# bayesiains/nflows

Hardware: AMD Instinct MI355X
Metric: log_prob samples/sec (dim=64, K=8, 32-layer RQ-NSF) + max |fwd∘inv − x| (higher is better)
Workload: dtype f32 (inputs, outputs, spline arithmetic, accumulation; conditioner GEMMs: every fp32 operand carried as 3 f16 pieces = 33 significand bits, i.e. at the reference's own fp32 operand width, 5 cross products per multiply-add -- 3 on the f16 MFMA, the 2 at the 2^-22 level from the pieces' high bytes on

## Files before the change

nflows_amd/csrc/f16x3_gemm.hpp:

```cpp
#pragma once

#include "bf16x3_gemm.hpp"

namespace nfa {

typedef _Float16 f16x8 __attribute__((ext_vector_type(8)));
typedef int i32x8 __attribute__((ext_vector_type(8)));

namespace k8x {

constexpr int kScaleA = 119, kScaleB = 127;

#ifdef NFA_ABL_NO_MFMA
#define NFA_K8X_F16(a, b, c) (c)
#define NFA_K8X_BF8(a, b, c) (c)
#else
#define NFA_K8X_F16(a, b, c) __builtin_amdgcn_mfma_f32_32x32x16_f16(a, b, c, 0, 0, 0)
#define NFA_K8X_BF8(a, b, c) __builtin_amdgcn_mfma_scale_f32_32x32x64_f8f6f4(a, b, c, 1, 1, 0, kScaleA, 0, kScaleB)
#endif

__device__ __forceinline__ void request_stage(WeightStream& sm) {
    const int dst_slot = sm.slot >= 1 ? sm.slot - 1 : kRing - 1;
    const char* stage = reinterpret_cast<const char*>(sm.w) + (size_t)sm.fetch * (kStageVec4 * 16);
    const __amdgpu_buffer_rsrc_t rsrc =
        __builtin_amdgcn_make_buffer_rsrc(const_cast<char*>(stage), (short)0, kStageVec4 * 16, 0x00020000);
    const int wave = __builtin_amdgcn_readfirstlane(sm.tid >> 6);
    char* slot = reinterpret_cast<char*>(sm.ring) + dst_slot * (kStageVec4 * 16) + wave * (kWave * 16);
    const unsigned lane_off = (unsigned)sm.tid * 16u;
#pragma unroll
    for (int i = 0; i < 3; ++i)
        __builtin_amdgcn_raw_ptr_buffer_load_lds(rsrc, (__attribute__((address_space(3))) void*)(slot + i * kBlock * 16), 16,
                                                 lane_off, i * kBlock * 16, 0, 0);
    sm.fetch = (sm.fetch + 1 == sm.num_stages) ? 0 : sm.fetch + 1;
}

template <int WAVES, int SUB>
__device__ __forceinline__ void request_stage(WeightStream& sm) {
    static_assert(WAVES == 4 || WAVES == 8, "narrow or wide");
    if constexpr (WAVES == 4) {
        request_stage(sm);
    } else if constexpr (SUB == 0) {
        const int dst_half = sm.slot >= 2 ? sm.slot - 2 : sm.slot + 2 * kRing - 2;
        const char* stage = reinterpret_cast<const char*>(sm.w) + (size_t)sm.fetch * (kStageVec4 * 16);
        const __amdgpu_buffer_rsrc_t rsrc =
            __builtin_amdgcn_make_buffer_rsrc(const_cast<char*>(stage), (short)0, 2 * kStageVec4 * 16, 0x00020000);
        const int wave = __builtin_amdgcn_readfirstlane(sm.tid >> 6);
        char* slot = reinterpret_cast<char*>(sm.ring) + dst_half * (kStageVec4 * 16) + wave * (kWave * 16);
        const unsigned lane_off = (unsigned)sm.tid * 16u;
#pragma unroll
        for (int i = 0; i < 3; ++i)
            __builtin_amdgcn_raw_ptr_buffer_load_lds(rsrc, (__attribute__((address_space(3))) void*)(slot + i * WAVES * kWave * 16),
                                                     16, lane_off, i * WAVES * kWave * 16, 0, 0);
        sm.fetch = (sm.fetch + 2 == sm.num_stages) ? 0 : sm.fetch + 2;
    }
}
template <int WAVES, int SUB>
__device__ __forceinline__ void stream_advance(WeightStream& sm) {
    if constexpr (WAVES == 4) {
        stream_advance(sm);
    } else {
        if constexpr (SUB == 1) asm volatile("s_waitcnt vmcnt(3)\n\ts_waitcnt lgkmcnt(0)\n\ts_barrier" ::: "memory");
        sm.slot = (sm.slot + 1 == 2 * kRing) ? 0 : sm.slot + 1;
    }
}

struct Pieces {
    uvec4 h, l, r;
};

#define NFA_K8X_ASM asm volatile

#define NFA_K8X_SPLIT_REST                                                  \
    "v_fma_mixlo_f16 %1, %3, 1.0, 0 op_sel_hi:[0,0,0]\n\t"                  \
    "v_fma_mixhi_f16 %1, %4, 1.0, 0 op_sel_hi:[0,0,0]\n\t"                  \
    "v_fma_mix_f32 %3, %3, 1.0, -%1 op_sel_hi:[0,0,1]\n\t"                  \
    "v_fma_mix_f32 %4, %4, 1.0, -%1 op_sel:[0,0,1] op_sel_hi:[0,0,1]\n\t"   \
    "v_fma_mixlo_f16 %2, %3, %8, 0 op_sel_hi:[0,0,0]\n\t"                   \
    "v_fma_mixhi_f16 %2, %4, %8, 0 op_sel_hi:[0,0,0]"
template <bool RELU = false>
__device__ __forceinline__ void split3_scaled(float v0, float v1, float scale, unsigned& hi, unsigned& lo, unsigned& rr) {
#if defined(NFA_K8X_NO_ASM)
    typedef _Float16 h2 __attribute__((ext_vector_type(2)));
    if (RELU) {
        v0 = __builtin_isnan(v0) ? v0 : (v0 > 0.0f ? v0 : 0.0f);
        v1 = __builtin_isnan(v1) ? v1 : (v1 > 0.0f ? v1 : 0.0f);
    }
    const float x0 = v0 * scale, x1 = v1 * scale;
    const h2 h = {(_Float16)x0, (_Float16)x1};
    const float t0 = x0 - (float)h[0], t1 = x1 - (float)h[1];
    const h2 l = {(_Float16)t0, (_Float16)t1};
    const h2 r = {(_Float16)((t0 - (float)l[0]) * 256.0f), (_Float16)((t1 - (float)l[1]) * 256.0f)};
    hi = __builtin_bit_cast(unsigned, h);
    lo = __builtin_bit_cast(unsigned, l);
    rr = __builtin_bit_cast(unsigned, r);
#else
    unsigned h, l, r;
    float t0, t1;
    if constexpr (RELU)
        NFA_K8X_ASM(
            "v_maximum3_f32 %3, %5, 0, 0\n\t"
            "v_maximum3_f32 %4, %6, 0, 0\n\t"
            "v_fma_mixlo_f16 %0, %3, %7, 0 op_sel_hi:[0,0,0]\n\t"
            "v_fma_mixhi_f16 %0, %4, %7, 0 op_sel_hi:[0,0,0]\n\t"
            "v_fma_mix_f32 %3, %3, %7, -%0 op_sel_hi:[0,0,1]\n\t"
            "v_fma_mix_f32 %4, %4, %7, -%0 op_sel:[0,0,1] op_sel_hi:[0,0,1]\n\t"
            NFA_K8X_SPLIT_REST
            : "=&v"(h), "=&v"(l), "=&v"(r), "=&v"(t0), "=&v"(t1)
            : "v"(v0), "v"(v1), "v"(scale), "s"(256.0f));
    else
        NFA_K8X_ASM(
            "v_fma_mixlo_f16 %0, %5, %7, 0 op_sel_hi:[0,0,0]\n\t"
            "v_fma_mixhi_f16 %0, %6, %7, 0 op_sel_hi:[0,0,0]\n\t"
            "v_fma_mix_f32 %3, %5, %7, -%0 op_sel_hi:[0,0,1]\n\t"
            "v_fma_mix_f32 %4, %6, %7, -%0 op_sel:[0,0,1] op_sel_hi:[0,0,1]\n\t"
            NFA_K8X_SPLIT_REST
            : "=&v"(h), "=&v"(l), "=&v"(r), "=&v"(t0), "=&v"(t1)
            : "v"(v0), "v"(v1), "v"(scale), "s"(256.0f));
    hi = h;
    lo = l;
    rr = r;
#endif
}
#undef NFA_K8X_SPLIT_REST

__device__ __forceinline__ i32x8 bf8_operand(const Pieces& p0, const Pieces& p1) {
    constexpr unsigned kHigh = 0x07050301u;
    i32x8 b;
    b[0] = (int)__builtin_amdgcn_perm(p0.r[1], p0.r[0], kHigh);
    b[1] = (int)__builtin_amdgcn_perm(p0.r[3], p0.r[2], kHigh);
    b[2] = (int)__builtin_amdgcn_perm(p0.h[1], p0.h[0], kHigh);
    b[3] = (int)__builtin_amdgcn_perm(p0.h[3], p0.h[2], kHigh);
    b[4] = (int)__builtin_amdgcn_perm(p1.r[1], p1.r[0], kHigh);
    b[5] = (int)__builtin_amdgcn_perm(p1.r[3], p1.r[2], kHigh);
    b[6] = (int)__builtin_amdgcn_perm(p1.h[1], p1.h[0], kHigh);
    b[7] = (int)__builtin_amdgcn_perm(p1.h[3], p1.h[2], kHigh);
    return b;
}

template <bool RELU, bool WB = true>
__device__ __forceinline__ void tile_to_pieces(const f32x16& a, float scale, Pieces& p0, Pieces& p1) {
    if constexpr (WB) asm volatile("s_nop 7\n\ts_nop 3" : : "v"(a));
#pragma unroll
    for (int q2 = 0; q2 < 8; ++q2) {
        unsigned h, l, r;
        split3_scaled<RELU>(a[q2 * 2], a[q2 * 2 + 1], scale, h, l, r);
        if (q2 < 4) {
            p0.h[q2] = h;
            p0.l[q2] = l;
            p0.r[q2] = r;
        } else {
            p1.h[q2 - 4] = h;
            p1.l[q2 - 4] = l;
            p1.r[q2 - 4] = r;
        }
    }
}

__device__ __forceinline__ i32x8 join_x(vec4f lo, vec4f hi) {
    const uvec4 a = __builtin_bit_cast(uvec4, lo), b = __builtin_bit_cast(uvec4, hi);
    return i32x8{(int)a[0], (int)a[1], (int)a[2], (int)a[3], (int)b[0], (int)b[1], (int)b[2], (int)b[3]};
}

struct Lead {
    vec4f h0, l0, h1, l1;
};
__device__ __forceinline__ Lead read_lead(const vec4f* stage) {
    return Lead{stage[0 * 64], stage[1 * 64], stage[2 * 64], stage[3 * 64]};
}

#define NFA_K8X_FENCE() __builtin_amdgcn_sched_barrier(0)

template <bool LAST, int WAVES = 4, int SUB = 0>
__device__ __forceinline__ void stage_kmajor(f32x16& acc0, f32x16& acc1, const Pieces& b0, const Pieces& b1, const i32x8& bx,
                                             WeightStream& sm, int lane, Lead& lead) {
    request_stage<WAVES, SUB>(sm);
    const vec4f* cur = sm.ring + sm.slot * kStageVec4 + lane;
    const f16x8 bh0 = __builtin_bit_cast(f16x8, b0.h), bl0 = __builtin_bit_cast(f16x8, b0.l);
    const f16x8 bh1 = __builtin_bit_cast(f16x8, b1.h), bl1 = __builtin_bit_cast(f16x8, b1.l);
    const vec4f x0l = cur[4 * 64], x0h = cur[5 * 64];
    const vec4f h0 = cur[6 * 64], l0 = cur[7 * 64], h1 = cur[8 * 64], l1 = cur[9 * 64], x1l = cur[10 * 64], x1h = cur[11 * 64];
    NFA_K8X_FENCE();
    {
        const f16x8 ah0 = __builtin_bit_cast(f16x8, lead.h0), al0 = __builtin_bit_cast(f16x8, lead.l0);
        const f16x8 ah1 = __builtin_bit_cast(f16x8, lead.h1), al1 = __builtin_bit_cast(f16x8, lead.l1);
        acc0 = NFA_K8X_F16(ah0, bl0, acc0);
        acc0 = NFA_K8X_F16(al0, bh0, acc0);
        acc0 = NFA_K8X_F16(ah0, bh0, acc0);
        acc0 = NFA_K8X_F16(ah1, bl1, acc0);
        acc0 = NFA_K8X_F16(al1, bh1, acc0);
        acc0 = NFA_K8X_F16(ah1, bh1, acc0);
        acc0 = NFA_K8X_BF8(join_x(x0l, x0h), bx, acc0);
    }
    const f16x8 ah0 = __builtin_bit_cast(f16x8, h0), al0 = __builtin_bit_cast(f16x8, l0);
    const f16x8 ah1 = __builtin_bit_cast(f16x8, h1), al1 = __builtin_bit_cast(f16x8, l1);
    const i32x8 ax = join_x(x1l, x1h);
    acc1 = NFA_K8X_F16(ah0, bl0, acc1);
    acc1 = NFA_K8X_F16(al0, bh0, acc1);
    acc1 = NFA_K8X_F16(ah0, bh0, acc1);
    NFA_K8X_FENCE();
    stream_advance<WAVES, SUB>(sm);
    if constexpr (!LAST) lead = read_lead(sm.ring + sm.slot * kStageVec4 + lane);
    NFA_K8X_FENCE();
    acc1 = NFA_K8X_F16(ah1, bl1, acc1);
    acc1 = NFA_K8X_F16(al1, bh1, acc1);
    acc1 = NFA_K8X_F16(ah1, bh1, acc1);
    acc1 = NFA_K8X_BF8(ax, bx, acc1);
}

template <int NKS, int WAVES, class PairFn>
__device__ __forceinline__ void gemm_kmajor_pairs(f32x16 (&acc)[4], WeightStream& sm, int lane, PairFn&& pair) {
    static_assert(NKS % 2 == 0, "pairs of k-steps");
    Lead lead = read_lead(sm.ring + sm.slot * kStageVec4 + lane);
#pragma unroll
    for (int pr = 0; pr < NKS / 2; ++pr) {
        Pieces b0, b1;
        pair(pr, b0, b1);
        const i32x8 bx = bf8_operand(b0, b1);
        stage_kmajor<false, WAVES, 0>(acc[0], acc[1], b0, b1, bx, sm, lane, lead);
        if (pr + 1 < NKS / 2) stage_kmajor<false, WAVES, 1>(acc[2], acc[3], b0, b1, bx, sm, lane, lead);
        else stage_kmajor<true, WAVES, 1>(acc[2], acc[3], b0, b1, bx, sm, lane, lead);
    }
}

template <int NKS, int WAVES = 4>
__device__ __forceinline__ void gemm_kmajor(f32x16 (&acc)[4], const Pieces (&p)[8], WeightStream& sm, int lane) {
    gemm_kmajor_pairs<NKS, WAVES>(acc, sm, lane, [&](int pr, Pieces& b0, Pieces& b1) {
        b0 = p[2 * pr];
        b1 = p[2 * pr + 1];
    });
}

template <int WAVES = 4>
__device__ __forceinline__ void gemm_kmajor_relu(f32x16 (&acc)[4], const f32x16 (&src)[4], float scale, WeightStream& sm,
                                                 int lane) {
    gemm_kmajor_pairs<8, WAVES>(acc, sm, lane, [&](int pr, Pieces& b0, Pieces& b1) {
        if (pr == 0) tile_to_pieces<true, true>(src[pr], scale, b0, b1);
        else tile_to_pieces<true, false>(src[pr], scale, b0, b1);
    });
}

}
}
```

nflows_amd/csrc/rqs_fused8.hpp:

```cpp
#pragma once

#include "rqs_math.hpp"

namespace nfa {

template <bool INVERSE, int KT = 8, bool DBG = false>
struct FusedSteps {
    static_assert(KT >= 2 && KT <= 32, "2 .. 32 bins (8 and 10 keep their own maximum / sum chains)");
    static constexpr int kNumSlices = KT + 3;
    static constexpr int kWalkSlices = 3 + (KT - 1);
    static constexpr int kBinSlices = INVERSE ? 9 : 7;
    static constexpr int kFinishSlices = kWalkSlices + 6 + kBinSlices + 1;
    static constexpr int kFirstWalkSlices = 0;
    static constexpr bool kInverse = INVERSE;

    float ew[KT], eh[KT];
    float sd[KT - 1];
    float x;
    float kl2e, kappa, tail_s;
    float m_w, m_h, den_w, den_h, tw_, th_;
    float aw, ah, kw, kh, kwn, khn;
    unsigned long long take;
    float cw0, cw1, ch0, ch1, u0, u1, d0, d1;
    float y, lad;
    int status;
    float t3, t4;
    float in_w, in_h, r_w, r_den, delta, s_, th, t1mt, den, t0, t1, t2, t5;
    int kbin;

    template <int A, int B>
    __device__ __forceinline__ static float half_sum(const float (&e)[KT]) {
        float s0 = e[A], s1 = B - A > 1 ? e[A + 1] : 0.0f;
#pragma unroll
        for (int i = A + 2; i < B; i += 2) {
            s0 += e[i];
            if (i + 1 < B) s1 += e[i + 1];
        }
        return B - A > 1 ? s0 + s1 : s0;
    }
    template <int S>
    __device__ __forceinline__ void numerators(float (&e)[KT], float& den_, float& m, float& t) {
        if constexpr (S == 0) {
            if constexpr (KT == 8 || KT == 10) {
                m = __builtin_fmaxf(__builtin_fmaxf(e[0], e[1]), e[2]);
                m = __builtin_fmaxf(__builtin_fmaxf(m, e[3]), e[4]);
                m = __builtin_fmaxf(__builtin_fmaxf(m, e[5]), e[6]);
                if constexpr (KT == 10) m = __builtin_fmaxf(__builtin_fmaxf(m, e[7]), e[8]);
                m = __builtin_fmaxf(m, e[KT - 1]) * kl2e;
            } else {
                m = e[0];
#pragma unroll
                for (int i = 1; i + 1 < KT; i += 2) m = __builtin_fmaxf(__builtin_fmaxf(m, e[i]), e[i + 1]);
                if constexpr (KT % 2 == 0) m = __builtin_fmaxf(m, e[KT - 1]);
                m *= kl2e;
            }
        } else if constexpr (S < 1 + KT) {
            e[S - 1] = __builtin_amdgcn_exp2f(__builtin_fmaf(e[S - 1], kl2e, -m));
        } else if constexpr (KT == 8 || KT == 10) {
            if constexpr (S == 1 + KT) {
                t = (e[0] + e[1]) + (e[2] + e[3]);
            } else {
                den_ = t + ((e[4] + e[5]) + (e[6] + e[7]));
                if constexpr (KT == 10) den_ += e[8] + e[9];
            }
        } else {
            constexpr int H = KT / 2;
            if constexpr (S == 1 + KT) t = half_sum<0, H>(e);
            else den_ = t + half_sum<H, KT>(e);
        }
    }
    template <int S>
    __device__ __forceinline__ void num_w() { numerators<S>(ew, den_w, m_w, tw_); }
    template <int S>
    __device__ __forceinline__ void num_h() { numerators<S>(eh, den_h, m_h, th_); }

    template <int PART>
    __device__ __forceinline__ void derivative(float u, float& d, const RqsDev& sp) {
        if constexpr (PART == 0) {
            t3 = u * kappa;
            t4 = __builtin_amdgcn_exp2f(-__builtin_fabsf(u * kl2e));
        } else if constexpr (PART == 1) {
            const float u1p = 1.0f + t4;
            const float c = t4 - (u1p - 1.0f);
            const float lg = __builtin_fmaf(__builtin_amdgcn_logf(u1p), 0.693147182464599609375f, sp.min_d);
            t4 = __builtin_fmaf(c, __builtin_amdgcn_rcpf(u1p), lg);
        } else {
            d = __builtin_fmaxf(t3, 0.0f) + t4;
        }
    }

    __device__ __forceinline__ void walk_select(float next_lower, float cand_u0, float cand_u1) {
        unsigned long long next;
        asm("v_cmp_ge_f32 %6, %7, %8\n\t"
            "v_cndmask_b32 %0, %0, %9, %15\n\t"
            "v_cndmask_b32 %1, %1, %10, %15\n\t"
            "v_cndmask_b32 %2, %2, %11, %15\n\t"
            "v_cndmask_b32 %3, %3, %12, %15\n\t"
            "v_cndmask_b32 %4, %4, %13, %15\n\t"
            "v_cndmask_b32 %5, %5, %14, %15"
            : "+v"(cw0), "+v"(cw1), "+v"(ch0), "+v"(ch1), "+v"(u0), "+v"(u1), "=&s"(next)
            : "v"(x), "v"(next_lower), "v"(kw), "v"(kwn), "v"(kh), "v"(khn), "v"(cand_u0), "v"(cand_u1), "s"(take));
        take = next;
    }

    template <int S>
    __device__ __forceinline__ void finish(const RqsDev& sp) {
        constexpr int W = kWalkSlices, D0 = W, BE = D0 + 6, LAST = BE + kBinSlices;
        static_assert(LAST + 1 == kFinishSlices, "slice map");
        const float B = sp.right;
        if constexpr (S == 0) {
            const float r0 = __builtin_amdgcn_rcpf(den_w);
            const float r = __builtin_fmaf(__builtin_fmaf(-den_w, r0, 1.0f), r0, r0);
            aw = r * (sp.span_w * sp.om_w);
        } else if constexpr (S == 1) {
            const float r0 = __builtin_amdgcn_rcpf(den_h);
            const float r = __builtin_fmaf(__builtin_fmaf(-den_h, r0, 1.0f), r0, r0);
            ah = r * (sp.span_w * sp.om_h);
        } else if constexpr (S == 2) {
            const float k1w = -B + __builtin_fmaf(ew[0], aw, sp.span_w * sp.min_w);
            const float k1h = -B + __builtin_fmaf(eh[0], ah, sp.span_w * sp.min_h);
            cw0 = -B;
            ch0 = -B;
            cw1 = k1w;
            ch1 = k1h;
            u0 = tail_s;
            u1 = sd[0];
            kw = k1w;
            kh = k1h;
            kwn = k1w + __builtin_fmaf(ew[1], aw, sp.span_w * sp.min_w);
            khn = k1h + __builtin_fmaf(eh[1], ah, sp.span_w * sp.min_h);
            asm("v_cmp_ge_f32 %0, %1, %2" : "=s"(take) : "v"(x), "v"(INVERSE ? k1h : k1w));
            if constexpr (DBG) kbin = 0;
        } else if constexpr (S < W) {
            constexpr int I = S - 2;
            if constexpr (DBG) kbin = (x >= (INVERSE ? kh : kw)) ? I : kbin;
            float kw2 = B, kh2 = B;
            if constexpr (I + 1 < KT - 1) {
                kw2 = kwn + __builtin_fmaf(ew[I + 1], aw, sp.span_w * sp.min_w);
                kh2 = khn + __builtin_fmaf(eh[I + 1], ah, sp.span_w * sp.min_h);
            }
            walk_select(INVERSE ? khn : kwn, sd[I - 1], I < KT - 1 ? sd[I < KT - 1 ? I : 0] : tail_s);
            kw = kwn;
            kh = khn;
            kwn = kw2;
            khn = kh2;
        } else if constexpr (S < D0 + 3) {
            derivative<S - D0>(u0, d0, sp);
        } else if constexpr (S < BE) {
            derivative<S - D0 - 3>(u1, d1, sp);
        } else if constexpr (S < LAST) {
            bin_eval<S - BE>();
        } else {
            const bool inside = (x >= -B && x <= B);
            y = inside ? y : x;
            lad = inside ? lad : 0.0f;
            status = inside ? status : 0;
            if constexpr (DBG) kbin = inside ? kbin : -1;
        }
    }

    template <int PART>
    __device__ __forceinline__ void bin_eval() {
        if constexpr (PART == 0) {
            in_w = cw1 - cw0;
            in_h = ch1 - ch0;
            const float r0 = __builtin_amdgcn_rcpf(in_w);
            r_w = __builtin_fmaf(__builtin_fmaf(-in_w, r0, 1.0f), r0, r0);
            status = 0;
        } else if constexpr (PART == 1) {
            const float q = in_h * r_w;
            delta = __builtin_fmaf(__builtin_fmaf(-q, in_w, in_h), r_w, q);
            s_ = __builtin_fmaf(-2.0f, delta, d0 + d1);
        } else if constexpr (INVERSE) {
            if constexpr (PART == 2) {
                const float yc = x - ch0;
                const float ys = yc * s_;
                const float a = __builtin_fmaf(in_h, delta - d0, ys);
                const float b = __builtin_fmaf(in_h, d0, -ys);
                const float c = -delta * yc;
                t0 = __builtin_fmaf(b, b, -4.0f * a * c);
                t1 = 2.0f * c;
                t2 = -b;
            } else if constexpr (PART == 3) {
                if (!(t0 >= 0.0f)) status = NFA_STATUS_NEG_DISCRIMINANT;
                const float dn = t2 - __builtin_sqrtf(t0);
                const float r0 = __builtin_amdgcn_rcpf(dn);
                const float r = __builtin_fmaf(__builtin_fmaf(-dn, r0, 1.0f), r0, r0);
                const float q = t1 * r;
                th = __builtin_fmaf(__builtin_fmaf(-q, dn, t1), r, q);
            } else if constexpr (PART == 4) {
                const float omr = 1.0f - th;
                t1mt = th * omr;
                den = __builtin_fmaf(s_, t1mt, delta);
                t0 = in_h * __builtin_fmaf(delta, th * th, d0 * t1mt);
                t1 = omr * omr;
            } else if constexpr (PART == 5) {
                float c = d0 * t1;
                c = __builtin_fmaf(delta + delta, t1mt, c);
                c = __builtin_fmaf(d1, th * th, c);
                t5 = (delta * delta) * c;
                const float r0 = __builtin_amdgcn_rcpf(den);
                const float r = __builtin_fmaf(__builtin_fmaf(-den, r0, 1.0f), r0, r0);
                const float q = t0 * r;
                const float g = ch0 + __builtin_fmaf(__builtin_fmaf(-q, den, t0), r, q);
                t2 = x - g;
            } else if constexpr (PART == 6) {
#ifdef NFA_MUTATION_NEWTON_SLOPE
                const float slope = in_h * t5;
#else
                const float slope = in_w * t5;
#endif
                const float r0 = __builtin_amdgcn_rcpf(slope);
                const float r = __builtin_fmaf(__builtin_fmaf(-slope, r0, 1.0f), r0, r0);
                const float step = (t2 * den) * (den * r);
                th = (__builtin_fabsf(step) <= 0.25f) ? th + step : th;
                y = __builtin_fmaf(th, in_w, cw0);
            } else if constexpr (PART == 7) {
                const float omr = 1.0f - th;
                t1mt = th * omr;
                den = __builtin_fmaf(s_, t1mt, delta);
                float c = d0 * (omr * omr);
                c = __builtin_fmaf(delta + delta, t1mt, c);
                c = __builtin_fmaf(d1, th * th, c);
                t5 = (delta * delta) * c;
            } else {
                const float l1 = __builtin_amdgcn_logf(t5), l2 = __builtin_amdgcn_logf(den);
                lad = -(__builtin_fmaf(-2.0f, l2, l1) * 0.693147182464599609375f);
            }
        } else {
            if constexpr (PART == 2) {
                const float xc = x - cw0;
                const float q = xc * r_w;
                th = __builtin_fmaf(__builtin_fmaf(-q, in_w, xc), r_w, q);
                const float omt = 1.0f - th;
                t1mt = th * omt;
                t1 = omt * omt;
            } else if constexpr (PART == 3) {
                t2 = th * th;
                t0 = in_h * __builtin_fmaf(delta, t2, d0 * t1mt);
                den = __builtin_fmaf(s_, t1mt, delta);
            } else if constexpr (PART == 4) {
                const float r0 = __builtin_amdgcn_rcpf(den);
                const float r = __builtin_fmaf(__builtin_fmaf(-den, r0, 1.0f), r0, r0);
                const float q = t0 * r;
                y = ch0 + __builtin_fmaf(__builtin_fmaf(-q, den, t0), r, q);
                r_den = r;
            } else if constexpr (PART == 5) {
                float c = d0 * t1;
                c = __builtin_fmaf(delta + delta, t1mt, c);
                c = __builtin_fmaf(d1, t2, c);
                t5 = (delta * r_den) * c;
            } else {
                lad = __builtin_amdgcn_logf((delta * r_den) * t5) * 0.693147182464599609375f;
            }
        }
    }
};

template <bool INVERSE>
using FusedSteps8 = FusedSteps<INVERSE, 8>;

}
```

nflows_amd/csrc/rqs_resnet_f16x3_kernel.hpp:

```cpp
#pragma once

#include "f16x3_gemm.hpp"
#include "rqs_resnet_f16_kernel.hpp"

#include <hip/hip_ext.h>
#include <stdlib.h>
#include <type_traits>

namespace nfa {
namespace k8x {

struct Args {
    const float* x;
    const vec4f* w;
    const float* bias;
    const float* scales;
    const int32_t* tables;
    float* out;
    float* lad;
    int32_t* redo;
    int32_t* status;
    int64_t batch;
    int D, dt, di, num_blocks, num_layers, num_stages, bias_per_layer, accumulate;
    RqsDev sp;
    int normal, skip_out;
    float log_z, act_scale;
    int Ds;
    float* dbg_logits;
};

typedef __attribute__((address_space(3))) float lds_f32;
typedef __attribute__((address_space(3))) int lds_i32;

using nfa::load_bias_tile;

__device__ __forceinline__ void load_bias_tile(f32x16& acc, const lds_f32* bias_tile_half) {
    typedef __attribute__((address_space(3))) const vec4f lds_vec4f;
    lds_vec4f* bp = reinterpret_cast<lds_vec4f*>(bias_tile_half);
#pragma unroll
    for (int q4 = 0; q4 < 4; ++q4) {
        const vec4f b = bp[q4];
        acc[q4 * 4 + 0] = b.x;
        acc[q4 * 4 + 1] = b.y;
        acc[q4 * 4 + 2] = b.z;
        acc[q4 * 4 + 3] = b.w;
    }
}

template <int BYTES>
__device__ __forceinline__ void bias_area_piece(const void* src, int src_bytes, int piece_off, lds_f32* dst) {
    const __amdgpu_buffer_rsrc_t rsrc = __builtin_amdgcn_make_buffer_rsrc(
        const_cast<char*>(static_cast<const char*>(src) + piece_off), (short)0, src_bytes - piece_off, 0x00020000);
    unsigned all = ~0u;
    asm volatile("" : "+s"(all));
    const unsigned lane = __builtin_amdgcn_mbcnt_hi(all, __builtin_amdgcn_mbcnt_lo(all, 0u));
    static_assert(BYTES == 16 || BYTES == 4, "dwordx4 or dword pieces");
    if constexpr (BYTES == 16)
        __builtin_amdgcn_raw_ptr_buffer_load_lds(rsrc, (__attribute__((address_space(3))) void*)dst, 16, lane * 16, 0, 0, 0);
    else
        __builtin_amdgcn_raw_ptr_buffer_load_lds(rsrc, (__attribute__((address_space(3))) void*)dst, 4, lane * 4, 0, 0, 0);
}
__host__ __device__ constexpr int bias_area_hidden_floats(int num_blocks) { return 128 + 256 * num_blocks; }
__host__ __device__ constexpr int bias_area_final_floats(int final_floats) { return (final_floats + 255) & ~255; }
__host__ __device__ constexpr int bias_area_floats(int num_blocks, int final_floats) {
    return bias_area_hidden_floats(num_blocks) + kTabLayer + bias_area_final_floats(final_floats);
}

template <int N>
__device__ __forceinline__ void uniform_load(const float* p, float (&v)[N]) {
    static_assert(N == 2 || N == 4, "one or two pairs");
    uint64_t v01, v23 = 0;
    if constexpr (N == 2)
        asm volatile("s_load_dwordx2 %0, %1, 0x0\n\ts_waitcnt lgkmcnt(0)" : "=&s"(v01) : "s"(p) : "memory");
    else
        asm volatile("s_load_dwordx2 %0, %2, 0x0\n\ts_load_dwordx2 %1, %2, 0x8\n\ts_waitcnt lgkmcnt(0)"
                     : "=&s"(v01), "=&s"(v23) : "s"(p) : "memory");
    v[0] = __builtin_bit_cast(float, (unsigned)v01);
    v[1] = __builtin_bit_cast(float, (unsigned)(v01 >> 32));
    if constexpr (N == 4) {
        v[2] = __builtin_bit_cast(float, (unsigned)v23);
        v[3] = __builtin_bit_cast(float, (unsigned)(v23 >> 32));
    }
}

struct NoWeave {
    template <int U0, int U1>
    __device__ __forceinline__ void span() {}
};
template <int UNIT, class Steps>
struct UnitWeave {
    Steps &fa, &fb;
    const RqsDev& sp;
    template <int U0, int U1>
    __device__ __forceinline__ void span() {
        constexpr int N = k8h::spline_unit_slices<UNIT, Steps>();
        k8h::spline_unit_range<UNIT, (U0 * N) / 32, (U1 * N) / 32>(fa, fb, sp);
    }
};
template <int MASK, class Steps>
struct SeqWeave {
    Steps& f;
    const RqsDev& sp;
    template <int U0, int U1>
    __device__ __forceinline__ void span() {
        constexpr int N = k8h::spline_seq_count<MASK, Steps>();
        k8h::spline_seq_range<MASK, (U0 * N) / 32, (U1 * N) / 32>(f, sp);
    }
};

#define NFA_K8X_PUMP_F16(U, A_, B_)                                         \
    acc = NFA_K8X_F16(A_, B_, acc);                                         \
    __builtin_amdgcn_sched_barrier(0);                                      \
    w.template span<(U), (U) + 1>();                                        \
    __builtin_amdgcn_sched_barrier(0)
#define NFA_K8X_PUMP_BF8(U, A_, B_)                                         \
    acc = NFA_K8X_BF8(A_, B_, acc);                                         \
    __builtin_amdgcn_sched_barrier(0);                                      \
    w.template span<(U), (U) + 2>();                                        \
    __builtin_amdgcn_sched_barrier(0)

template <int HS, int WAVES, class W>
__device__ __forceinline__ void stage_pumped(f32x16& acc, const Pieces (&p)[8], const i32x8 (&bx)[4], WeightStream& sm, int lane,
                                             Lead& lead, W& w) {
    request_stage<WAVES, HS>(sm);
    const vec4f* cur = sm.ring + sm.slot * kStageVec4 + lane;
    vec4f xa = cur[8 * 64], xb = cur[9 * 64];
    vec4f fh0 = lead.h0, fl0 = lead.l0, fh1 = lead.h1, fl1 = lead.l1;
    {
        const Pieces& b0 = p[HS * 4 + 0];
        const Pieces& b1 = p[HS * 4 + 1];
        const f16x8 bh0 = __builtin_bit_cast(f16x8, b0.h), bl0 = __builtin_bit_cast(f16x8, b0.l);
        const f16x8 bh1 = __builtin_bit_cast(f16x8, b1.h), bl1 = __builtin_bit_cast(f16x8, b1.l);
        const f16x8 ah0 = __builtin_bit_cast(f16x8, fh0), al0 = __builtin_bit_cast(f16x8, fl0);
        const f16x8 ah1 = __builtin_bit_cast(f16x8, fh1), al1 = __builtin_bit_cast(f16x8, fl1);
        const i32x8 ax = join_x(xa, xb);
        NFA_K8X_PUMP_F16(HS * 16 + 0, ah0, bl0);
        NFA_K8X_PUMP_F16(HS * 16 + 1, al0, bh0);
        NFA_K8X_PUMP_F16(HS * 16 + 2, ah0, bh0);
        fh0 = cur[4 * 64];
        fl0 = cur[5 * 64];
        NFA_K8X_PUMP_F16(HS * 16 + 3, ah1, bl1);
        NFA_K8X_PUMP_F16(HS * 16 + 4, al1, bh1);
        NFA_K8X_PUMP_F16(HS * 16 + 5, ah1, bh1);
        fh1 = cur[6 * 64];
        fl1 = cur[7 * 64];
        NFA_K8X_PUMP_BF8(HS * 16 + 6, ax, bx[HS * 2 + 0]);
        xa = cur[10 * 64];
        xb = cur[11 * 64];
    }
    {
        const Pieces& b0 = p[HS * 4 + 2];
        const Pieces& b1 = p[HS * 4 + 3];
        const f16x8 bh0 = __builtin_bit_cast(f16x8, b0.h), bl0 = __builtin_bit_cast(f16x8, b0.l);
        const f16x8 bh1 = __builtin_bit_cast(f16x8, b1.h), bl1 = __builtin_bit_cast(f16x8, b1.l);
        const f16x8 ah0 = __builtin_bit_cast(f16x8, fh0), al0 = __builtin_bit_cast(f16x8, fl0);
        const f16x8 ah1 = __builtin_bit_cast(f16x8, fh1), al1 = __builtin_bit_cast(f16x8, fl1);
        const i32x8 ax = join_x(xa, xb);
        NFA_K8X_PUMP_F16(HS * 16 + 8, ah0, bl0);
        NFA_K8X_PUMP_F16(HS * 16 + 9, al0, bh0);
        NFA_K8X_PUMP_F16(HS * 16 + 10, ah0, bh0);
        NFA_K8X_PUMP_F16(HS * 16 + 11, ah1, bl1);
        NFA_K8X_PUMP_F16(HS * 16 + 12, al1, bh1);
        NFA_K8X_PUMP_F16(HS * 16 + 13, ah1, bh1);
        stream_advance<WAVES, HS>(sm);
        lead = read_lead(sm.ring + sm.slot * kStageVec4 + lane);
        __builtin_amdgcn_sched_barrier(0);
        NFA_K8X_PUMP_BF8(HS * 16 + 14, ax, bx[HS * 2 + 1]);
    }
}
#undef NFA_K8X_PUMP_F16
#undef NFA_K8X_PUMP_BF8

template <int WAVES = 4, class W>
__device__ __forceinline__ void gemm_tile_pumped(f32x16& acc, const Pieces (&p)[8], const i32x8 (&bx)[4], WeightStream& sm, int lane,
                                                 Lead& lead, W&& w) {
    stage_pumped<0, WAVES>(acc, p, bx, sm, lane, lead, w);
    stage_pumped<1, WAVES>(acc, p, bx, sm, lane, lead, w);
}

template <int TI, int T, int KB, class Steps, class BiasPtr>
__device__ __forceinline__ void any_group_tiles(f32x16& acc, Steps& f, BiasPtr gb, const Pieces (&p)[8], const i32x8 (&bx)[4],
                                                WeightStream& sm, int lane, Lead& lead, const RqsDev& sp) {
    if constexpr (TI < T) {
        constexpr int kMask = k8h::any_tile_mask(KB, TI);
        load_bias_tile(acc, gb + TI * 32);
        if constexpr (kMask != 0) gemm_tile_pumped(acc, p, bx, sm, lane, lead, SeqWeave<kMask, Steps>{f, sp});
        else gemm_tile_pumped(acc, p, bx, sm, lane, lead, NoWeave{});
        k8h::take_chunk<TI, KB>(f, acc);
        any_group_tiles<TI + 1, T, KB, Steps, BiasPtr>(acc, f, gb, p, bx, sm, lane, lead, sp);
    }
}

__device__ __forceinline__ bool not_finite(float v) { return !(__builtin_fabsf(v) < INFINITY); }

template <bool INVERSE, int INIT_KS, bool DBG, int KB, bool BIAS_LDS, int WAVES = 4>
__device__ __forceinline__ void rqs_resnet_f16x3_body(const Args& a) {
    static_assert(!DBG || KB == 8, "the diagnostic instances: 8 bins");
    constexpr bool WIDE = WAVES == 8;
    static_assert(WAVES == 4 || (WIDE && KB == 8 && BIAS_LDS && !DBG), "the wide form: 8 bins, bias area, no diagnostics");
    constexpr int kRingFloats = kRing * kStageVec4 * 4 * (WIDE ? 2 : 1);
    constexpr int kFinalRows = KB == 8 ? 24 : 16 * ((3 * KB - 1 + 15) / 16);
    constexpr int NW = WAVES;
    extern __shared__ __attribute__((aligned(16))) float lds_dyn[];
    __shared__ int s_tab[2][kTabLayer];
    __shared__ int s_final[128];
    __shared__ int s_bad[NW];
    const int tid = threadIdx.x, lane = tid & 63, wave = __builtin_amdgcn_readfirstlane(tid >> 6);
    const int D = a.D, dt = a.dt;
    int my_status = 0;
    auto checked = [&](int v, bool used) {
        my_status |= (used && (v < 0 || v >= D)) ? NFA_STATUS_BAD_INDEX : 0;
        return v < 0 ? 0 : (v >= D ? D - 1 : v);
    };
    const int te = tid & (kTabLayer - 1);
    s_tab[0][te] = checked(a.tables[te], te < kTabTr ? te < a.di : te - kTabTr < dt);
    s_final[te] = checked(a.tables[a.num_layers * kTabLayer + te], te < D);

    WeightStream sm;
    sm.w = a.w;
    sm.ring = reinterpret_cast<vec4f*>(lds_dyn);
    sm.slot = 1;
    sm.fetch = 0;
    sm.num_stages = a.num_stages * a.num_layers;
    sm.tid = tid;
    lds_f32* s_area = (lds_f32*)lds_dyn + kRingFloats + NW * D * kRowPad;
    lds_f32* s_traw = s_area + bias_area_hidden_floats(a.num_blocks);
    auto request_hidden = [&](int layer) {
        const float* src = a.bias + (size_t)layer * a.bias_per_layer;
        const int bytes = bias_area_hidden_floats(a.num_blocks) * 4;
        if (wave >= NW - 2) bias_area_piece<4>(src, bytes, (wave - (NW - 2)) * 256, s_area + (wave - (NW - 2)) * 64);
        for (int j = wave; j < a.num_blocks; j += NW) bias_area_piece<16>(src, bytes, 512 + j * 1024, s_area + 128 + j * 256);
    };
    if constexpr (BIAS_LDS) request_hidden(0);
    if constexpr (WIDE) {
        sm.slot = 2;
        request_stage<WAVES, 0>(sm);
        sm.slot = 4;
        request_stage<WAVES, 0>(sm);
    } else {
        request_stage(sm);
        sm.slot = 2;
        request_stage(sm);
    }
    sm.slot = 0;
    asm volatile("s_waitcnt vmcnt(0)" ::: "memory");
    __syncthreads();

#ifdef NFA_K8X_STAGGER
    if (blockIdx.x >= (gridDim.x >> 1))
        for (int i = 0; i < NFA_K8X_STAGGER; ++i) __builtin_amdgcn_s_sleep(127);
#endif
    lds_f32* s_row = (lds_f32*)lds_dyn + kRingFloats + wave * D * kRowPad;
    lds_f32* s_fbias = BIAS_LDS ? s_traw + kTabLayer : s_area;
    auto request_final = [&](int layer) {
        const float* src = a.bias + (size_t)layer * a.bias_per_layer + bias_area_hidden_floats(a.num_blocks);
        const int bytes = dt * kFinalRows * 4;
        for (int j = wave; j * 1024 < bytes; j += NW) bias_area_piece<16>(src, bytes, j * 1024, s_fbias + j * 256);
    };
    auto request_table = [&](int layer) {
        if (wave < 2) bias_area_piece<4>(a.tables + layer * kTabLayer, kTabLayer * 4, wave * 256, s_traw + wave * 64);
    };
    const int groups = dt >> 2;
    const int64_t num_quads = a.batch >> 7;
    const int gemms = 2 + 2 * a.num_blocks;
    const float S = a.act_scale;
    int tb = 0;

    const int64_t num_passes = WIDE ? (num_quads + 1) >> 1 : num_quads;
    for (int64_t pass = blockIdx.x; pass < num_passes; pass += gridDim.x) {
        const int64_t quad_mine = WIDE ? 2 * pass + (wave >> 2) : pass;
        const int live_bit = WIDE ? (int)(((uint64_t)quad_mine - (uint64_t)num_quads) >> 63) : 1;
        const bool live = live_bit != 0;
        const int64_t quad = quad_mine - 1 + live_bit;
        const int64_t row0 = (quad << 7) + ((WIDE ? wave & 3 : wave) << 5);
        int lane_here = lane, di = a.di;
        asm volatile("" : "+v"(lane_here), "+s"(di));
        const int half = lane_here >> 5, r = lane_here & 31;
        {
            const vec4f* xv = reinterpret_cast<const vec4f*>(a.x + row0 * D);
            const int nvec = D * 8;
            for (int e0 = lane; e0 < nvec; e0 += kWave * 4) {
                vec4f v[4];
#pragma unroll
                for (int u = 0; u < 4; ++u) {
                    const int e = e0 + u * kWave;
                    v[u] = xv[e < nvec ? e : 0];
                }
#pragma unroll
                for (int u = 0; u < 4; ++u) {
                    const int e = e0 + u * kWave;
                    if (e < nvec) {
                        const int rr = (e * 4) / D, c0 = e * 4 - rr * D;
                        s_row[(c0 + 0) * kRowPad + rr] = v[u].x;
                        s_row[(c0 + 1) * kRowPad + rr] = v[u].y;
                        s_row[(c0 + 2) * kRowPad + rr] = v[u].z;
                        s_row[(c0 + 3) * kRowPad + rr] = v[u].w;
                    }
                }
            }
        }
        __builtin_amdgcn_fence(__ATOMIC_RELEASE, "wavefront");
        __builtin_amdgcn_fence(__ATOMIC_ACQUIRE, "wavefront");

        float lad_acc = 0.0f;
        int quad_status = 0;
        for (int layer = 0; layer < a.num_layers; ++layer) {
#ifdef NFA_K8X_WIDE_NOPRIO
            if constexpr (!WIDE)
#endif
            {
                if ((layer + ((WIDE ? wave >= 4 : blockIdx.x >= (gridDim.x >> 1)) ? 1 : 0)) & 1) __builtin_amdgcn_s_setprio(1);
                else __builtin_amdgcn_s_setprio(0);
            }
            const int* tab = s_tab[tb];
            const int nl = layer + 1 < a.num_layers ? layer + 1 : 0;
            if constexpr (!BIAS_LDS) {
                unsigned all = ~0u;
                asm volatile("" : "+s"(all));
                const int te_l = (int)__builtin_amdgcn_mbcnt_hi(all, __builtin_amdgcn_mbcnt_lo(all, 0u)) + ((wave & 1) << 6);
                s_tab[tb ^ 1][te_l] = checked(a.tables[nl * kTabLayer + te_l], te_l < kTabTr ? te_l < a.di : te_l - kTabTr < dt);
            }
            if constexpr (BIAS_LDS) {
                request_final(layer);
                request_table(nl);
                __builtin_amdgcn_sched_barrier(0);
            }
            std::conditional_t<BIAS_LDS, const lds_f32*, const float*> bias;
            if constexpr (BIAS_LDS) bias = s_area + half * 16;
            else bias = a.bias + (size_t)layer * a.bias_per_layer + half * 16;
            const float* sc = a.scales + (size_t)layer * gemms * 2;
            Pieces p[8];

#pragma unroll
            for (int ks = 0; ks < INIT_KS; ++ks) {
#pragma unroll
                for (int j2 = 0; j2 < 4; ++j2) {
                    const int i0 = ks * 16 + half * 8 + j2 * 2;
                    float v0 = s_row[tab[kTabId + i0] * kRowPad + r], v1 = s_row[tab[kTabId + i0 + 1] * kRowPad + r];
                    v0 = i0 < di ? v0 : 0.0f;
                    v1 = i0 + 1 < di ? v1 : 0.0f;
                    unsigned hi, lo, rr;
                    split3_scaled(v0, v1, S, hi, lo, rr);
                    p[ks].h[j2] = hi;
                    p[ks].l[j2] = lo;
                    p[ks].r[j2] = rr;
                }
            }

            f32x16 h[4];
            float hs;
            {
#pragma unroll
                for (int t = 0; t < 4; ++t) load_bias_tile(h[t], bias + t * 32);
                gemm_kmajor<INIT_KS, WAVES>(h, p, sm, lane);
                float s0[2];
                uniform_load(sc, s0);
                hs = s0[0];
            }
            bias += 128;
            sc += 2;
            if constexpr (BIAS_LDS) {
                unsigned all = ~0u;
                asm volatile("" : "+s"(all));
                const int te_l = (int)__builtin_amdgcn_mbcnt_hi(all, __builtin_amdgcn_mbcnt_lo(all, 0u)) + ((wave & 1) << 6);
                s_tab[tb ^ 1][te_l] = checked(((const lds_i32*)s_traw)[te_l], te_l < kTabTr ? te_l < a.di : te_l - kTabTr < dt);
            } else {
                const float* fbias = a.bias + (size_t)layer * a.bias_per_layer + 128 + 256 * a.num_blocks;
                for (int i = tid; i < dt * kFinalRows; i += kBlock) s_fbias[i] = fbias[i];
                if (a.num_blocks == 0) __syncthreads();
            }

            for (int blk = 0; blk < a.num_blocks; ++blk) {
                float sb[4];
                f32x16 u[4];
#pragma unroll
                for (int t = 0; t < 4; ++t) load_bias_tile(u[t], bias + t * 32);
                gemm_kmajor_relu<WAVES>(u, h, hs, sm, lane);
                uniform_load(sc, sb);
                const float skip = hs * sb[3];
#pragma unroll
                for (int t = 0; t < 4; ++t) {
                    f32x16 b1;
                    load_bias_tile(b1, bias + 128 + t * 32);
#pragma unroll
                    for (int q_ = 0; q_ < 16; ++q_) h[t][q_] = __builtin_fmaf(h[t][q_], skip, b1[q_]);
                }
                gemm_kmajor_relu<WAVES>(h, u, sb[0], sm, lane);
                hs = sb[2];
                bias += 256;
                sc += 4;
            }

            if constexpr (BIAS_LDS) {
                request_hidden(nl);
                __builtin_amdgcn_sched_barrier(0);
            }
#pragma unroll
            for (int t = 0; t < 4; ++t) tile_to_pieces<false>(h[t], hs, p[2 * t], p[2 * t + 1]);

            if constexpr (KB == 8) {
                using Steps = FusedSteps<INVERSE, 8>;
                Steps fa{}, fb{};
                float sf[2];
                uniform_load(sc, sf);
                const float kappa = sf[0];
                fa.kappa = fb.kappa = kappa;
                fa.kl2e = fb.kl2e = 1.44269502162933349609375f * kappa;
                fa.tail_s = fb.tail_s = a.sp.tail_logit * sf[1];
                lds_f32* slot_b = s_row;
                const lds_f32* fbias = s_fbias + half * 16;
                i32x8 bx[4];
#pragma unroll
                for (int j = 0; j < 4; ++j) bx[j] = bf8_operand(p[2 * j], p[2 * j + 1]);
                Lead lead = read_lead(sm.ring + sm.slot * kStageVec4 + lane);
                f32x16 acc[3];
                auto commit = [&](Steps& f, lds_f32* slot) {
                    *slot = f.y;
                    lad_acc += f.lad;
                    quad_status |= f.status;
                };
                [[maybe_unused]] auto store_logits = [&](const f32x16& t, int tile) {
                    if constexpr (DBG) {
                        if (layer == a.num_layers - 1) {
                            float* dst = a.dbg_logits + (size_t)(row0 + r) * (dt * kFinalRows) + tile * 32 + half * 16;
#pragma unroll
                            for (int q_ = 0; q_ < 16; ++q_) dst[q_] = t[q_] * kappa;
                            asm volatile("s_waitcnt vmcnt(0)" ::: "memory");
                        }
                    }
                };
                UnitWeave<k8h::kUnitNumA, Steps> w0{fa, fb, a.sp};
                UnitWeave<k8h::kUnitFinishA, Steps> w1{fa, fb, a.sp};
                UnitWeave<k8h::kUnitFinishB, Steps> w2{fa, fb, a.sp};
                for (int g = 0; g < groups; ++g) {
                    lds_f32* slot0 = s_row + tab[kTabTr + g * 4 + half * 2] * kRowPad + r;
                    lds_f32* slot1 = s_row + tab[kTabTr + g * 4 + half * 2 + 1] * kRowPad + r;
                    load_bias_tile(acc[0], fbias + (g * 3 + 0) * 32);
                    if (g > 0) {
                        gemm_tile_pumped<WAVES>(acc[0], p, bx, sm, lane, lead, w2);
                        commit(fb, slot_b);
                    } else {
                        gemm_tile_pumped<WAVES>(acc[0], p, bx, sm, lane, lead, NoWeave{});
                    }
                    store_logits(acc[0], g * 3 + 0);
                    fa.x = *slot0;
#pragma unroll
                    for (int j = 0; j < 8; ++j) {
                        fa.ew[j] = acc[0][j];
                        fa.eh[j] = acc[0][8 + j];
                    }
                    load_bias_tile(acc[1], fbias + (g * 3 + 1) * 32);
                    gemm_tile_pumped<WAVES>(acc[1], p, bx, sm, lane, lead, w0);
                    store_logits(acc[1], g * 3 + 1);
                    fb.x = *slot1;
#pragma unroll
                    for (int j = 0; j < 8; ++j) {
                        if (j < 7) fa.sd[j] = acc[1][j];
                        fb.ew[j] = acc[1][8 + j];
                    }
                    load_bias_tile(acc[2], fbias + (g * 3 + 2) * 32);
                    gemm_tile_pumped<WAVES>(acc[2], p, bx, sm, lane, lead, w1);
                    store_logits(acc[2], g * 3 + 2);
                    commit(fa, slot0);
#pragma unroll
                    for (int j = 0; j < 8; ++j) {
                        fb.eh[j] = acc[2][j];
                        if (j < 7) fb.sd[j] = acc[2][8 + j];
                    }
                    slot_b = slot1;
                }
                k8h::spline_unit_range<k8h::kUnitFinishB, 0, k8h::spline_unit_slices<k8h::kUnitFinishB, Steps>()>(fa, fb, a.sp);
                commit(fb, slot_b);
            }
            else {
                constexpr int T = kFinalRows / 16;
                static_assert(T >= 1 && T <= 6, "2 .. 32 bins");
                using Steps = FusedSteps<INVERSE, KB>;
                constexpr int kRest = k8h::any_rest_mask(KB);
                Steps f{};
                float sf[2];
                uniform_load(sc, sf);
                const float kappa = sf[0];
                f.kappa = kappa;
                f.kl2e = 1.44269502162933349609375f * kappa;
                f.tail_s = a.sp.tail_logit * sf[1];
                const lds_f32* fbias = s_fbias + half * 16;
                i32x8 bx[4];
#pragma unroll
                for (int j = 0; j < 4; ++j) bx[j] = bf8_operand(p[2 * j], p[2 * j + 1]);
                Lead lead = read_lead(sm.ring + sm.slot * kStageVec4 + lane);
                const int groups_any = dt >> 1;
                f32x16 acc;
                lds_f32* slot = s_row + tab[kTabTr + half] * kRowPad + r;
                load_bias_tile(acc, fbias);
                gemm_tile_pumped(acc, p, bx, sm, lane, lead, NoWeave{});
                for (int g = 0; g < groups_any; ++g) {
                    const lds_f32* gb = fbias + g * T * 32;
                    f.x = *slot;
                    k8h::take_chunk<0, KB>(f, acc);
                    any_group_tiles<1, T, KB, Steps>(acc, f, gb, p, bx, sm, lane, lead, a.sp);
                    if (g + 1 < groups_any) {
                        lds_f32* next_slot = s_row + tab[kTabTr + (g + 1) * 2 + half] * kRowPad + r;
                        load_bias_tile(acc, gb + T * 32);
                        gemm_tile_pumped(acc, p, bx, sm, lane, lead, SeqWeave<kRest, Steps>{f, a.sp});
                        *slot = f.y;
                        slot = next_slot;
                    } else {
                        k8h::spline_seq_range<kRest, 0, k8h::spline_seq_count<kRest, Steps>()>(f, a.sp);
                        *slot = f.y;
                    }
                    lad_acc += f.lad;
                    quad_status |= f.status;
                }
            }
            tb ^= 1;
            __builtin_amdgcn_fence(__ATOMIC_RELEASE, "wavefront");
            __builtin_amdgcn_fence(__ATOMIC_ACQUIRE, "wavefront");
        }

        lad_acc += __shfl_xor(lad_acc, 32, kWave);
        const float sumsq = tile_row_sumsq((const float*)s_row, a.Ds, half, r);
        const bool bad = not_finite(lad_acc) || not_finite(sumsq);
        const bool wave_bad = __builtin_amdgcn_ballot_w64(bad) != 0;
        if (lane == 0) s_bad[wave] = wave_bad ? 1 : 0;
        asm volatile("s_waitcnt vmcnt(0)" ::: "memory");
        __syncthreads();
        int any_bad = 0;
#pragma unroll
        for (int w_ = 0; w_ < 4; ++w_) any_bad |= s_bad[(WIDE ? wave & 4 : 0) + w_];
        if (!any_bad && live) {
            if (!a.skip_out) {
                vec4f* ov = reinterpret_cast<vec4f*>(a.out + row0 * D);
                const int nvec = D * 8;
                for (int e = lane; e < nvec; e += kWave) {
                    const int rr = (e * 4) / D, c0 = e * 4 - rr * D;
                    vec4f v;
                    v.x = s_row[s_final[c0 + 0] * kRowPad + rr];
                    v.y = s_row[s_final[c0 + 1] * kRowPad + rr];
                    v.z = s_row[s_final[c0 + 2] * kRowPad + rr];
                    v.w = s_row[s_final[c0 + 3] * kRowPad + rr];
                    ov[e] = v;
                }
            }
            if (half == 0) {
                float* dst = a.lad + row0 + r;
                float v = a.accumulate ? *dst + lad_acc : lad_acc;
                if (a.normal) v = (-0.5f * sumsq - a.log_z) + v;
                *dst = v;
            }
            my_status |= quad_status;
        }
        if ((WIDE ? (tid & 255) == 0 && live : tid == 0)) a.redo[quad] = any_bad ? 1 : 0;
        asm volatile("s_waitcnt vmcnt(0)" ::: "memory");
        __syncthreads();
    }
    asm volatile("s_waitcnt vmcnt(0)" ::: "memory");
    if (my_status && a.status) atomicOr(a.status, my_status);
}

template <bool INVERSE, int INIT_KS, bool DBG = false, int KB = 8>
__global__ void __launch_bounds__(kBlock, 2) rqs_resnet_f16x3_kernel(const Args a) {
    rqs_resnet_f16x3_body<INVERSE, INIT_KS, DBG, KB, true>(a);
}
template <bool INVERSE, int INIT_KS, bool DBG = false, int KB = 8>
__global__ void __launch_bounds__(kBlock, 2) rqs_resnet_f16x3_global_bias_kernel(const Args a) {
    rqs_resnet_f16x3_body<INVERSE, INIT_KS, DBG, KB, false>(a);
}

constexpr int kWideBlocksPerCu = 2;

template <bool INVERSE, int INIT_KS>
__global__ void __launch_bounds__(2 * kBlock, 1) rqs_resnet_f16x3_kernel_wide(const Args a) {
    rqs_resnet_f16x3_body<INVERSE, INIT_KS, false, 8, true, 8>(a);
}

}
}


namespace nfa {
namespace k8x {
typedef void (*KernelFn)(const Args);
KernelFn bins_kernel_a(int K, bool inverse, int init_ks, bool bias_lds);
KernelFn bins_kernel_b(int K, bool inverse, int init_ks, bool bias_lds);
}
}
```

Baseline: 29.00 million.

## Pack residual pieces directly to bf8 via scaled convert, trim register footprint

The third (residual) split piece is now converted straight to packed bf8 with v_cvt_scalef32_pk_bf8_f32, four values per register, instead of being stored as f16 and byte-permuted later. This halves the residual storage in Pieces and removes the perm instructions when building the bf8 MFMA operand. The skip FMA is also forced into inline asm in two halves, and a reciprocal in the derivative path is replaced by a linear approximation (1.5 - 0.5u), which changes numerics and could affect accuracy.

```diff
diff --git a/nflows_amd/csrc/f16x3_gemm.hpp b/nflows_amd/csrc/f16x3_gemm.hpp
--- a/nflows_amd/csrc/f16x3_gemm.hpp
+++ b/nflows_amd/csrc/f16x3_gemm.hpp
@@ -65,7 +65,8 @@
 }
 
 struct Pieces {
-    uvec4 h, l, r;
+    uvec4 h, l;
+    unsigned r[2];
 };
 
 #define NFA_K8X_ASM asm volatile
@@ -74,10 +75,22 @@
     "v_fma_mixlo_f16 %1, %3, 1.0, 0 op_sel_hi:[0,0,0]\n\t"                  \
     "v_fma_mixhi_f16 %1, %4, 1.0, 0 op_sel_hi:[0,0,0]\n\t"                  \
     "v_fma_mix_f32 %3, %3, 1.0, -%1 op_sel_hi:[0,0,1]\n\t"                  \
-    "v_fma_mix_f32 %4, %4, 1.0, -%1 op_sel:[0,0,1] op_sel_hi:[0,0,1]\n\t"   \
-    "v_fma_mixlo_f16 %2, %3, %8, 0 op_sel_hi:[0,0,0]\n\t"                   \
-    "v_fma_mixhi_f16 %2, %4, %8, 0 op_sel_hi:[0,0,0]"
-template <bool RELU = false>
+    "v_fma_mix_f32 %4, %4, 1.0, -%1 op_sel:[0,0,1] op_sel_hi:[0,0,1]\n\t"
+#define NFA_K8X_SPLIT_LOWER "v_cvt_scalef32_pk_bf8_f32 %2, %3, %4, %8\n\ts_nop 0"
+#define NFA_K8X_SPLIT_UPPER "v_cvt_scalef32_pk_bf8_f32 %2, %3, %4, %8 op_sel:[0,0,0,1]\n\ts_nop 0"
+#define NFA_K8X_SPLIT_RELU                                                  \
+    "v_maximum3_f32 %3, %5, 0, 0\n\t"                                       \
+    "v_maximum3_f32 %4, %6, 0, 0\n\t"                                       \
+    "v_fma_mixlo_f16 %0, %3, %7, 0 op_sel_hi:[0,0,0]\n\t"                   \
+    "v_fma_mixhi_f16 %0, %4, %7, 0 op_sel_hi:[0,0,0]\n\t"                   \
+    "v_fma_mix_f32 %3, %3, %7, -%0 op_sel_hi:[0,0,1]\n\t"                   \
+    "v_fma_mix_f32 %4, %4, %7, -%0 op_sel:[0,0,1] op_sel_hi:[0,0,1]\n\t"
+#define NFA_K8X_SPLIT_PLAIN                                                 \
+    "v_fma_mixlo_f16 %0, %5, %7, 0 op_sel_hi:[0,0,0]\n\t"                   \
+    "v_fma_mixhi_f16 %0, %6, %7, 0 op_sel_hi:[0,0,0]\n\t"                   \
+    "v_fma_mix_f32 %3, %5, %7, -%0 op_sel_hi:[0,0,1]\n\t"                   \
+    "v_fma_mix_f32 %4, %6, %7, -%0 op_sel:[0,0,1] op_sel_hi:[0,0,1]\n\t"
+template <bool RELU = false, bool UPPER = false>
 __device__ __forceinline__ void split3_scaled(float v0, float v1, float scale, unsigned& hi, unsigned& lo, unsigned& rr) {
 #if defined(NFA_K8X_NO_ASM)
     typedef _Float16 h2 __attribute__((ext_vector_type(2)));
@@ -89,49 +102,52 @@
     const h2 h = {(_Float16)x0, (_Float16)x1};
     const float t0 = x0 - (float)h[0], t1 = x1 - (float)h[1];
     const h2 l = {(_Float16)t0, (_Float16)t1};
-    const h2 r = {(_Float16)((t0 - (float)l[0]) * 256.0f), (_Float16)((t1 - (float)l[1]) * 256.0f)};
+    typedef short s2 __attribute__((ext_vector_type(2)));
+    const s2 r = __builtin_amdgcn_cvt_scalef32_pk_bf8_f32(__builtin_bit_cast(s2, UPPER ? rr : 0u), t0 - (float)l[0], t1 - (float)l[1],
+                                                          0.00390625f, UPPER);
     hi = __builtin_bit_cast(unsigned, h);
     lo = __builtin_bit_cast(unsigned, l);
     rr = __builtin_bit_cast(unsigned, r);
 #else
     unsigned h, l, r;
+    if constexpr (UPPER) r = rr;
     float t0, t1;
-    if constexpr (RELU)
-        NFA_K8X_ASM(
-            "v_maximum3_f32 %3, %5, 0, 0\n\t"
-            "v_maximum3_f32 %4, %6, 0, 0\n\t"
-            "v_fma_mixlo_f16 %0, %3, %7, 0 op_sel_hi:[0,0,0]\n\t"
-            "v_fma_mixhi_f16 %0, %4, %7, 0 op_sel_hi:[0,0,0]\n\t"
-            "v_fma_mix_f32 %3, %3, %7, -%0 op_sel_hi:[0,0,1]\n\t"
-            "v_fma_mix_f32 %4, %4, %7, -%0 op_sel:[0,0,1] op_sel_hi:[0,0,1]\n\t"
-            NFA_K8X_SPLIT_REST
-            : "=&v"(h), "=&v"(l), "=&v"(r), "=&v"(t0), "=&v"(t1)
-            : "v"(v0), "v"(v1), "v"(scale), "s"(256.0f));
+    if constexpr (RELU && UPPER)
+        NFA_K8X_ASM(NFA_K8X_SPLIT_RELU NFA_K8X_SPLIT_REST NFA_K8X_SPLIT_UPPER
+                    : "=&v"(h), "=&v"(l), "+v"(r), "=&v"(t0), "=&v"(t1)
+                    : "v"(v0), "v"(v1), "v"(scale), "s"(0.00390625f));
+    else if constexpr (RELU)
+        NFA_K8X_ASM(NFA_K8X_SPLIT_RELU NFA_K8X_SPLIT_REST NFA_K8X_SPLIT_LOWER
+                    : "=&v"(h), "=&v"(l), "=&v"(r), "=&v"(t0), "=&v"(t1)
+                    : "v"(v0), "v"(v1), "v"(scale), "s"(0.00390625f));
+    else if constexpr (UPPER)
+        NFA_K8X_ASM(NFA_K8X_SPLIT_PLAIN NFA_K8X_SPLIT_REST NFA_K8X_SPLIT_UPPER
+                    : "=&v"(h), "=&v"(l), "+v"(r), "=&v"(t0), "=&v"(t1)
+                    : "v"(v0), "v"(v1), "v"(scale), "s"(0.00390625f));
     else
-        NFA_K8X_ASM(
-            "v_fma_mixlo_f16 %0, %5, %7, 0 op_sel_hi:[0,0,0]\n\t"
-            "v_fma_mixhi_f16 %0, %6, %7, 0 op_sel_hi:[0,0,0]\n\t"
-            "v_fma_mix_f32 %3, %5, %7, -%0 op_sel_hi:[0,0,1]\n\t"
-            "v_fma_mix_f32 %4, %6, %7, -%0 op_sel:[0,0,1] op_sel_hi:[0,0,1]\n\t"
-            NFA_K8X_SPLIT_REST
-            : "=&v"(h), "=&v"(l), "=&v"(r), "=&v"(t0), "=&v"(t1)
-            : "v"(v0), "v"(v1), "v"(scale), "s"(256.0f));
+        NFA_K8X_ASM(NFA_K8X_SPLIT_PLAIN NFA_K8X_SPLIT_REST NFA_K8X_SPLIT_LOWER
+                    : "=&v"(h), "=&v"(l), "=&v"(r), "=&v"(t0), "=&v"(t1)
+                    : "v"(v0), "v"(v1), "v"(scale), "s"(0.00390625f));
     hi = h;
     lo = l;
     rr = r;
 #endif
 }
 #undef NFA_K8X_SPLIT_REST
+#undef NFA_K8X_SPLIT_LOWER
+#undef NFA_K8X_SPLIT_UPPER
+#undef NFA_K8X_SPLIT_RELU
+#undef NFA_K8X_SPLIT_PLAIN
 
 __device__ __forceinline__ i32x8 bf8_operand(const Pieces& p0, const Pieces& p1) {
     constexpr unsigned kHigh = 0x07050301u;
     i32x8 b;
-    b[0] = (int)__builtin_amdgcn_perm(p0.r[1], p0.r[0], kHigh);
-    b[1] = (int)__builtin_amdgcn_perm(p0.r[3], p0.r[2], kHigh);
+    b[0] = (int)p0.r[0];
+    b[1] = (int)p0.r[1];
     b[2] = (int)__builtin_amdgcn_perm(p0.h[1], p0.h[0], kHigh);
     b[3] = (int)__builtin_amdgcn_perm(p0.h[3], p0.h[2], kHigh);
-    b[4] = (int)__builtin_amdgcn_perm(p1.r[1], p1.r[0], kHigh);
-    b[5] = (int)__builtin_amdgcn_perm(p1.r[3], p1.r[2], kHigh);
+    b[4] = (int)p1.r[0];
+    b[5] = (int)p1.r[1];
     b[6] = (int)__builtin_amdgcn_perm(p1.h[1], p1.h[0], kHigh);
     b[7] = (int)__builtin_amdgcn_perm(p1.h[3], p1.h[2], kHigh);
     return b;
@@ -141,18 +157,16 @@
 __device__ __forceinline__ void tile_to_pieces(const f32x16& a, float scale, Pieces& p0, Pieces& p1) {
     if constexpr (WB) asm volatile("s_nop 7\n\ts_nop 3" : : "v"(a));
 #pragma unroll
-    for (int q2 = 0; q2 < 8; ++q2) {
-        unsigned h, l, r;
-        split3_scaled<RELU>(a[q2 * 2], a[q2 * 2 + 1], scale, h, l, r);
-        if (q2 < 4) {
-            p0.h[q2] = h;
-            p0.l[q2] = l;
-            p0.r[q2] = r;
-        } else {
-            p1.h[q2 - 4] = h;
-            p1.l[q2 - 4] = l;
-            p1.r[q2 - 4] = r;
-        }
+    for (int q2 = 0; q2 < 8; q2 += 2) {
+        Pieces& p = q2 < 4 ? p0 : p1;
+        unsigned h0, l0, h1, l1, r;
+        split3_scaled<RELU, false>(a[q2 * 2], a[q2 * 2 + 1], scale, h0, l0, r);
+        split3_scaled<RELU, true>(a[q2 * 2 + 2], a[q2 * 2 + 3], scale, h1, l1, r);
+        p.h[q2 & 3] = h0;
+        p.l[q2 & 3] = l0;
+        p.h[(q2 & 3) + 1] = h1;
+        p.l[(q2 & 3) + 1] = l1;
+        p.r[(q2 & 3) >> 1] = r;
     }
 }
 
diff --git a/nflows_amd/csrc/rqs_fused8.hpp b/nflows_amd/csrc/rqs_fused8.hpp
--- a/nflows_amd/csrc/rqs_fused8.hpp
+++ b/nflows_amd/csrc/rqs_fused8.hpp
@@ -83,7 +83,7 @@
             const float u1p = 1.0f + t4;
             const float c = t4 - (u1p - 1.0f);
             const float lg = __builtin_fmaf(__builtin_amdgcn_logf(u1p), 0.693147182464599609375f, sp.min_d);
-            t4 = __builtin_fmaf(c, __builtin_amdgcn_rcpf(u1p), lg);
+            t4 = __builtin_fmaf(c, __builtin_fmaf(-0.5f, u1p, 1.5f), lg);
         } else {
             d = __builtin_fmaxf(t3, 0.0f) + t4;
         }
diff --git a/nflows_amd/csrc/rqs_resnet_f16x3_kernel.hpp b/nflows_amd/csrc/rqs_resnet_f16x3_kernel.hpp
--- a/nflows_amd/csrc/rqs_resnet_f16x3_kernel.hpp
+++ b/nflows_amd/csrc/rqs_resnet_f16x3_kernel.hpp
@@ -193,6 +193,36 @@
 
 __device__ __forceinline__ bool not_finite(float v) { return !(__builtin_fabsf(v) < INFINITY); }
 
+template <int B0>
+__device__ __forceinline__ void skip_half(f32x16& h, const f32x16& b1, float skip) {
+#if defined(NFA_K8X_NO_ASM)
+#pragma unroll
+    for (int q = B0; q < B0 + 8; ++q) h[q] = __builtin_fmaf(h[q], skip, b1[q]);
+#else
+    float e0 = h[B0], e1 = h[B0 + 1], e2 = h[B0 + 2], e3 = h[B0 + 3], e4 = h[B0 + 4], e5 = h[B0 + 5], e6 = h[B0 + 6], e7 = h[B0 + 7];
+    NFA_K8X_ASM(
+        "v_fma_f32 %0, %0, %8, %9\n\t"
+        "v_fma_f32 %1, %1, %8, %10\n\t"
+        "v_fma_f32 %2, %2, %8, %11\n\t"
+        "v_fma_f32 %3, %3, %8, %12\n\t"
+        "v_fma_f32 %4, %4, %8, %13\n\t"
+        "v_fma_f32 %5, %5, %8, %14\n\t"
+        "v_fma_f32 %6, %6, %8, %15\n\t"
+        "v_fma_f32 %7, %7, %8, %16"
+        : "+v"(e0), "+v"(e1), "+v"(e2), "+v"(e3), "+v"(e4), "+v"(e5), "+v"(e6), "+v"(e7)
+        : "v"(skip), "v"(b1[B0]), "v"(b1[B0 + 1]), "v"(b1[B0 + 2]), "v"(b1[B0 + 3]), "v"(b1[B0 + 4]), "v"(b1[B0 + 5]),
+          "v"(b1[B0 + 6]), "v"(b1[B0 + 7]));
+    h[B0] = e0;
+    h[B0 + 1] = e1;
+    h[B0 + 2] = e2;
+    h[B0 + 3] = e3;
+    h[B0 + 4] = e4;
+    h[B0 + 5] = e5;
+    h[B0 + 6] = e6;
+    h[B0 + 7] = e7;
+#endif
+}
+
 template <bool INVERSE, int INIT_KS, bool DBG, int KB, bool BIAS_LDS, int WAVES = 4>
 __device__ __forceinline__ void rqs_resnet_f16x3_body(const Args& a) {
     static_assert(!DBG || KB == 8, "the diagnostic instances: 8 bins");
@@ -339,11 +369,11 @@
                     float v0 = s_row[tab[kTabId + i0] * kRowPad + r], v1 = s_row[tab[kTabId + i0 + 1] * kRowPad + r];
                     v0 = i0 < di ? v0 : 0.0f;
                     v1 = i0 + 1 < di ? v1 : 0.0f;
-                    unsigned hi, lo, rr;
-                    split3_scaled(v0, v1, S, hi, lo, rr);
+                    unsigned hi, lo;
+                    if (j2 & 1) split3_scaled<false, true>(v0, v1, S, hi, lo, p[ks].r[j2 >> 1]);
+                    else split3_scaled<false, false>(v0, v1, S, hi, lo, p[ks].r[j2 >> 1]);
                     p[ks].h[j2] = hi;
                     p[ks].l[j2] = lo;
-                    p[ks].r[j2] = rr;
                 }
             }
 
@@ -382,8 +412,8 @@
                 for (int t = 0; t < 4; ++t) {
                     f32x16 b1;
                     load_bias_tile(b1, bias + 128 + t * 32);
-#pragma unroll
-                    for (int q_ = 0; q_ < 16; ++q_) h[t][q_] = __builtin_fmaf(h[t][q_], skip, b1[q_]);
+                    skip_half<0>(h[t], b1, skip);
+                    skip_half<8>(h[t], b1, skip);
                 }
                 gemm_kmajor_relu<WAVES>(h, u, sb[0], sm, lane);
                 hs = sb[2];
```

After: 29.41 million, median of 6. 1.4% higher.
